# potamides/DeTikZify

Hardware: NVIDIA H100
Metric: TikZ tokens/sec/GPU (decode, 384px cond, 2k ctx) (higher is better)
Workload: dtype bf16

## Files before the change

### detikzify_b200/csrc/decode_mega.cu

```cuda
#include "common.cuh"
#include "fp8.cuh"
#include "launch.h"

namespace dtk {
namespace {

constexpr int NCW = 8;
constexpr int NPW = 4;
constexpr int MEGA_THREADS = (NCW + NPW) * 32;
constexpr int CONSUMER_THREADS = NCW * 32;
static_assert(NCW % NPW == 0, "slot ownership: NPW must divide NCW");
constexpr int TILE_BYTES = 8192;
constexpr int KV_V_OFF = 4096;
constexpr int NT = 104;
constexpr int NS = 72;
constexpr int NG = 48;
constexpr long long SPIN_CYCLES = 4000000000ll;

DTK_DEV void mbar_init(uint32_t bar, uint32_t count) {
  asm volatile("mbarrier.init.shared::cta.b64 [%0], %1;\n" ::"r"(bar), "r"(count));
}
DTK_DEV void mbar_expect_tx(uint32_t bar, uint32_t bytes) {
  asm volatile("mbarrier.arrive.expect_tx.shared::cta.b64 _, [%0], %1;\n" ::"r"(bar), "r"(bytes) : "memory");
}
DTK_DEV void mbar_arrive(uint32_t bar) {
  asm volatile("mbarrier.arrive.shared::cta.b64 _, [%0];\n" ::"r"(bar) : "memory");
}
DTK_DEV uint32_t mbar_try(uint32_t bar, uint32_t parity) {
  uint32_t done;
  asm volatile(
      "{\n\t.reg .pred p;\n\t"
      "mbarrier.try_wait.parity.shared::cta.b64 p, [%1], %2;\n\t"
      "selp.u32 %0, 1, 0, p;\n\t}\n"
      : "=r"(done)
      : "r"(bar), "r"(parity)
      : "memory");
  return done;
}
DTK_DEV void mbar_wait_slow(uint32_t bar, uint32_t parity) {
  uint32_t spins = 0;
  long long t0 = 0;
  while (!mbar_try(bar, parity)) {
    if ((++spins & 1023u) == 0) {
      const long long now = clock64();
      if (t0 == 0) t0 = now;
      else if (now - t0 > SPIN_CYCLES) __trap();
    }
  }
}
DTK_DEV void mbar_wait(uint32_t bar, uint32_t parity) {
  if (!mbar_try(bar, parity)) mbar_wait_slow(bar, parity);
}
DTK_DEV void bulk_g2s(uint32_t dst, const void* src, uint32_t bytes, uint32_t bar) {
  asm volatile("cp.async.bulk.shared::cluster.global.mbarrier::complete_tx::bytes [%0], [%1], %2, [%3];\n" ::"r"(dst),
               "l"(src), "r"(bytes), "r"(bar)
               : "memory");
}
DTK_DEV void bulk_g2s_hint(uint32_t dst, const void* src, uint32_t bytes, uint32_t bar, uint64_t pol) {
  asm volatile("cp.async.bulk.shared::cluster.global.mbarrier::complete_tx::bytes.L2::cache_hint [%0], [%1], %2, [%3], %4;\n" ::"r"(dst),
               "l"(src), "r"(bytes), "r"(bar), "l"(pol)
               : "memory");
}
DTK_DEV uint64_t policy_evict_first() {
  uint64_t pol;
  asm volatile("createpolicy.fractional.L2::evict_first.b64 %0, 1.0;\n" : "=l"(pol));
  return pol;
}
DTK_DEV void consumer_sync() { asm volatile("bar.sync 1, %0;\n" ::"n"(CONSUMER_THREADS) : "memory"); }

typedef unsigned long long u64;
DTK_DEV void st_tag(u64* p, float v, uint32_t tag) {
  const u64 w = ((u64)tag << 32) | (u64)__float_as_uint(v);
  asm volatile("st.relaxed.gpu.global.u64 [%0], %1;\n" ::"l"(p), "l"(w) : "memory");
}
DTK_DEV ulonglong2 ld_strong2(const u64* p) {
  ulonglong2 r;
  asm volatile("ld.relaxed.gpu.global.v2.u64 {%0, %1}, [%2];\n" : "=l"(r.x), "=l"(r.y) : "l"(p) : "memory");
  return r;
}
DTK_DEV ulonglong2 ld_weak2(const u64* p) {
  ulonglong2 r;
  asm volatile("ld.global.cg.v2.u64 {%0, %1}, [%2];\n" : "=l"(r.x), "=l"(r.y) : "l"(p) : "memory");
  return r;
}
DTK_DEV u64 ld_strong1(const u64* p) {
  u64 r;
  asm volatile("ld.relaxed.gpu.global.u64 %0, [%1];\n" : "=l"(r) : "l"(p) : "memory");
  return r;
}
DTK_DEV u64 ld_weak1(const u64* p) {
  u64 r;
  asm volatile("ld.global.cg.u64 %0, [%1];\n" : "=l"(r) : "l"(p) : "memory");
  return r;
}
DTK_DEV bool tag_ok(u64 w, uint32_t tag) { return (uint32_t)(w >> 32) == tag; }
DTK_DEV float tag_val(u64 w) { return __uint_as_float((uint32_t)w); }
struct Spin {
  uint32_t n = 0;
  long long t0 = 0;
  DTK_DEV void tick() {
    __nanosleep(32);
    if ((++n & 255u) == 0) {
      const long long now = clock64();
      if (t0 == 0) t0 = now;
      else if (now - t0 > SPIN_CYCLES) __trap();
    }
  }
};
DTK_DEV u64 poll1(const u64* p, uint32_t tag) {
  Spin sp;
  for (;;) {
    const u64 w = ld_strong1(p);
    if (tag_ok(w, tag)) return w;
    sp.tick();
  }
}
DTK_DEV float settle1(u64 w, const u64* p, uint32_t tag, bool nowait) {
  if (!tag_ok(w, tag) && !nowait) w = poll1(p, tag);
  return tag_val(w);
}

template <int N>
DTK_DEV void ld_pairs(const u64* const (&ptr)[N], const bool (&on)[N], uint32_t tag, bool nowait, float2 (&out)[N]) {
  ulonglong2 w[N];
#pragma unroll
  for (int u = 0; u < N; ++u)
    if (on[u]) w[u] = ld_weak2(ptr[u]);
  Spin sp;
  for (;;) {
    bool bad[N], any = false;
#pragma unroll
    for (int u = 0; u < N; ++u) {
      bad[u] = on[u] && !(tag_ok(w[u].x, tag) && tag_ok(w[u].y, tag));
      any = any || bad[u];
    }
    if (!any || nowait) break;
    sp.tick();
#pragma unroll
    for (int u = 0; u < N; ++u)
      if (bad[u]) w[u] = ld_strong2(ptr[u]);
  }
#pragma unroll
  for (int u = 0; u < N; ++u) out[u] = on[u] ? make_float2(tag_val(w[u].x), tag_val(w[u].y)) : make_float2(0.f, 0.f);
}

enum { PH_QKV = 0, PH_ATTN = 1, PH_O = 2, PH_GU = 3, PH_DOWN = 4, PH_LM = 5 };

struct AttnSplit {
  int active, head, j0, j1, last;
  int cph;
  int n_items;
// ... 50 lines not shown
        if (bad[u]) w[u] = ld_strong2(src + 2 * (ks * 128 + u * 32 + lane));
    }
#pragma unroll
    for (int u = 0; u < 4; ++u) v[u] = on[u] ? make_float2(tag_val(w[u].x), tag_val(w[u].y)) : make_float2(0.f, 0.f);
  } else {
#pragma unroll
    for (int u = 0; u < 4; ++u) {
      v[u] = make_float2(0.f, 0.f);
      if (on[u]) {
        const uint32_t e = *reinterpret_cast<const uint32_t*>(src_bf16 + 2 * (ks * 128 + u * 32 + lane));
        v[u] = make_float2(__uint_as_float(e << 16), __uint_as_float(e & 0xffff0000u));
      }
    }
  }
  float ss = 0.f;
#pragma unroll
  for (int u = 0; u < 4; ++u) {
    float a = v[u].x, b = v[u].y;
    if (norm_w) {
      ss += a * a + b * b;
      a *= __uint_as_float(gw[u] << 16);
      b *= __uint_as_float(gw[u] & 0xffff0000u);
    }
    const float ah = __bfloat162float(__float2bfloat16_rn(a)), bh = __bfloat162float(__float2bfloat16_rn(b));
    const uint32_t hi = pack_bf16x2(ah, bh), lo = pack_bf16x2(a - ah, b - bh);
    const uint32_t hi2 = __shfl_xor_sync(0xffffffffu, hi, 4), lo2 = __shfl_xor_sync(0xffffffffu, lo, 4);
    if (!(lane & 4)) xb[(size_t)(ks * 16 + u * 4 + (lane >> 3)) * 4 + (lane & 3)] = make_uint4(hi, hi2, lo, lo2);
  }
  if (norm_w) {
    ss = warp_sum(ss);
    if (lane == 0) slice_ss[ks] = ss;
  }
  __syncwarp();
  if (lane == 0) {
    __threadfence_block();
    slice_tag[ks] = my_tag;
  }
  __syncwarp();
}
DTK_DEV float slices_rn(const float* slice_ss, int nslice, int K, float eps) {
  const int lane = threadIdx.x & 31;
  float t = 0.f;
  for (int i = lane; i < nslice; i += 32) t += *reinterpret_cast<const volatile float*>(slice_ss + i);
  t = warp_sum(t);
  return rsqrtf(t / K + eps);
}

template <bool DBG, int HD, bool F8>
__global__ void __launch_bounds__(MEGA_THREADS, 1) decode_mega_kernel(const MegaArgs p) {
  constexpr int HALF = HD / 2;
  constexpr int LPK = HD / 8;
  constexpr int NGRP = 32 / LPK;
  constexpr int NST = NCW * NGRP;
  constexpr int PS = HD + 4;
  constexpr int PPL = HD / 64;
  constexpr int HSH = HD == 128 ? 7 : 6;
  extern __shared__ __align__(128) uint8_t smem[];
  const int tid = threadIdx.x, lane = tid & 31, warp = tid >> 5;
  const int c = blockIdx.x, G = gridDim.x;
  const int nslots = p.nslots;
  uint8_t* ring = smem;
  float* actf = reinterpret_cast<float*>(smem + (size_t)nslots * TILE_BYTES);
  uint4* xb = reinterpret_cast<uint4*>(actf);
  uint64_t* bars = reinterpret_cast<uint64_t*>(actf + p.act_floats);
  float* red = reinterpret_cast<float*>(bars + 2 * nslots);
  float* rope_s = red + 16;
  float* tpart = rope_s + 128;
  int* gcnt = reinterpret_cast<int*>(tpart + NT * 16);
  float* rbuf = reinterpret_cast<float*>(gcnt + NG);
  float* qkn = rbuf + NG * 16;
  float* slice_ss = qkn + 384;
  uint32_t* slice_tag = reinterpret_cast<uint32_t*>(slice_ss + NS);
  const uint32_t full0 = smem_u32(bars), empty0 = smem_u32(bars + nslots);
  const uint32_t ring_u32 = smem_u32(ring);

  if (tid == 0) {
    for (int s = 0; s < nslots; ++s) {
      mbar_init(full0 + 8 * s, 1);
      mbar_init(empty0 + 8 * s, 1);
    }
    asm volatile("fence.mbarrier_init.release.cluster;\n" ::: "memory");
    asm volatile("fence.proxy.async.shared::cta;\n" ::: "memory");
  }
  const int pos = p.pos[0], slot = p.slots[0];
  int tok = p.tok[0];
  if (tok < 0 || tok >= p.V) tok = 0;
  const int qd = p.heads * HD, kd = p.kv_heads * HD;
  if (tid < NS) slice_tag[tid] = (uint32_t)p.bar_base[1];
  if (tid < HD) rope_s[tid] = p.rope_cs[(int64_t)pos * HD + tid];
  __syncthreads();
  const AttnSplit as = attn_split(p, c, G, pos);
  const int kvh = as.head / (p.heads / p.kv_heads);
  const bf16* kv_slot = p.kv + (int64_t)slot * p.kv_slot_stride;
  const int shlen = p.share_len[0];
  const bf16* kv_share = p.kv + (int64_t)p.share_slot[0] * p.kv_slot_stride;
  const int nphase = 5 * p.L + 1;

  struct Walk {
    uint32_t nb = 0;
    uint32_t gb = 0;
    uint32_t rot = 0;
  };
  auto phase_span = [&](const Walk& w, const MegaMat& m, int& g0, int& cnt, int& nact) {
    nact = m.nact;
    int ci = c + G - (int)w.rot;
    if (ci >= G) ci -= G;
    g0 = ci * m.per;
    cnt = (ci < nact) ? min(m.per, m.groups - g0) : 0;
  };
  auto mat_of = [](int ph) { return ph == PH_QKV ? 0 : ph == PH_O ? 1 : ph == PH_GU ? 2 : ph == PH_DOWN ? 3 : 4; };

  if (warp >= NCW) {
    asm volatile("setmaxnreg.dec.sync.aligned.u32 56;\n");
    const uint32_t pw = (uint32_t)(warp - NCW);
    if (lane == 0) {
      const bool evf = !(p.variant & 1);
      const uint64_t pol = policy_evict_first();
      Walk w;
      uint32_t sl = pw, use = 0;
      long long* tr = nullptr;
      uint32_t tr_nb0 = 0;
      int l = 0, ph = 0;
      for (int it = 0; it < nphase; ++it) {
        if (it == nphase - 1) { ph = PH_LM; l = 0; }
        if (DBG && ph == 0) {
          tr = (p.dbg2 && l == p.dbg_layer && it != nphase - 1) ? p.dbg2 + (int64_t)c * MEGA_DBG2_ROWS * 4 : nullptr;
          if (tr) tr_nb0 = w.nb;
        }
        const bool attn = ph == PH_ATTN;
        const MegaMat& m = p.mat[mat_of(ph)];
        int g0 = 0, cnt = 0, nact = 0;
        if (!attn) phase_span(w, m, g0, cnt, nact);
        const int tpg = attn ? 1 : m.tpg;
        const int ntiles = attn ? as.n_items : cnt * tpg;
        const int64_t kvo = (int64_t)l * p.kv_layer_stride + (int64_t)kvh * p.max_len * HD;
        const bf16* base = attn ? kv_slot + kvo
                                : m.base + (int64_t)l * m.layer_stride + (int64_t)g0 * tpg * MEGA_TILE_ELEMS;
        uint32_t j = (pw + NPW - (w.nb & (NPW - 1))) & (NPW - 1);
        MegaF8 f8{};
        uint32_t jk = 0, jks = j;
        if (F8) {
          if (!attn && ph != PH_LM) f8 = p.f8[mat_of(ph)];
          while (jks >= (uint32_t)tpg) { jks -= tpg; ++jk; }
        }
        if ((int)j < ntiles) {
          for (; (int)j < ntiles; j += NPW) {
            if (use > 0) mbar_wait(empty0 + 8 * sl, (use - 1) & 1);
            const uint32_t dst = ring_u32 + sl * TILE_BYTES, fb = full0 + 8 * sl;
            if (attn) {
              const int key0 = as.j0 + (int)j * 16;
              const uint32_t bytes = (uint32_t)min(16, p.max_len - key0) * (uint32_t)(HD * 2);
              const bf16* kb = (key0 < shlen ? kv_share + kvo : base) + (int64_t)key0 * HD;
              mbar_expect_tx(fb, 2 * bytes);
              bulk_g2s(dst, kb, bytes, fb);
              bulk_g2s(dst + KV_V_OFF, kb + p.kv_v_offset, bytes, fb);
            } else if (F8 && ph != PH_LM) {
              mbar_expect_tx(fb, MEGA_F8_TILE_BYTES + 16);
              const uint8_t* src = f8.tiles + (int64_t)l * f8.layer_stride + ((int64_t)g0 * tpg + j) * MEGA_F8_TILE_BYTES;
              if (evf) bulk_g2s_hint(dst, src, MEGA_F8_TILE_BYTES, fb, pol);
              else bulk_g2s(dst, src, MEGA_F8_TILE_BYTES, fb);
              bulk_g2s(dst + MEGA_F8_TILE_BYTES, f8.exps + (int64_t)l * f8.exp_stride + (int64_t)(g0 + (int)jk) * 16, 16, fb);
            } else {
              mbar_expect_tx(fb, TILE_BYTES);
              if (evf) bulk_g2s_hint(dst, base + (int64_t)j * MEGA_TILE_ELEMS, TILE_BYTES, fb, pol);
              else bulk_g2s(dst, base + (int64_t)j * MEGA_TILE_ELEMS, TILE_BYTES, fb);
            }
            if (DBG && tr) {
              const uint32_t row = w.nb + j - tr_nb0;
              if (row < 160u) tr[row * 4] = clock64();
            }
            sl += NPW;
            if (sl >= (uint32_t)nslots) { sl -= nslots; ++use; }
            if (F8) {
              jks += NPW;
              while (jks >= (uint32_t)tpg) { jks -= tpg; ++jk; }
            }
          }
        }
        w.nb += ntiles;
        if (!attn) {
          w.gb += cnt;
          w.rot += (uint32_t)nact;
          if (w.rot >= (uint32_t)G) w.rot -= G;
        }
        if (++ph == 5) { ph = 0; ++l; }
      }
    }
    return;
  }

  asm volatile("setmaxnreg.inc.sync.aligned.u32 224;\n");
  const int dflags = DBG ? p.dbg_flags : 0;
  const bool nowait = (dflags & 2) != 0;
  unsigned long long bar_target = p.bar_base[0];
  const uint32_t epoch = (uint32_t)p.bar_base[1];
  Walk w;
  uint32_t sl = (uint32_t)warp, use = 0;
  uint32_t cur_slot = 0;
  auto release = [&]() {
    __syncwarp();
    if (lane == 0) mbar_arrive(empty0 + 8 * cur_slot);
  };
  long long* dbg = (DBG && p.dbg) ? p.dbg + (int64_t)c * nphase * 4 : nullptr;
  long long* ctr = nullptr;
  uint32_t ctr_nb0 = 0;
  int it = 0, l = 0, ph = 0;
  auto stamp = [&](int k) {
    if (!DBG) return;
    if (dbg && tid == 0) {
      unsigned long long t;
      asm volatile("mov.u64 %0, %%globaltimer;\n" : "=l"(t));
      dbg[it * 4 + k] = (long long)t;
    }
    if (ctr && tid == 0 && ph < 5) ctr[(160 + ph) * 4 + k] = clock64();
  };

  u64* const t_xa = p.tg;
  u64* const t_xb = t_xa + p.tg_H;
  u64* const t_q = t_xb + p.tg_H;
  u64* const t_kn = t_q + qd;
  u64* const t_vn = t_kn + kd;
  u64* const t_att = t_vn + kd;
  u64* const t_h = t_att + qd;
  u64* const t_part = t_h + p.tg_I;

  float best_v = -INFINITY;
  int best_i = 0x7fffffff;
  for (it = 0; it < nphase; ++it) {
    if (it == nphase - 1) { ph = PH_LM; l = 0; }
    const uint32_t tag = epoch + (uint32_t)it + 1u;
    if (DBG && ph == 0) {
      ctr = (p.dbg2 && l == p.dbg_layer && it != nphase - 1) ? p.dbg2 + (int64_t)c * MEGA_DBG2_ROWS * 4 : nullptr;
      ctr_nb0 = w.nb;
    }
    stamp(0);
    if (ph == PH_ATTN) {
      if (as.active) {
        const int hw = lane >> (HSH - 3), l16 = lane & (LPK - 1);
        if (warp == 0) {
          const float sl2 = (HD == 128 ? 0.08838834764831845f : 0.125f) * 1.4426950408889634f;
          float2* q2 = reinterpret_cast<float2*>(qkn);
          const bool lastr = as.last != 0;
          const u64* ptr[3 * PPL];
          bool on[3 * PPL];
#pragma unroll
          for (int u = 0; u < PPL; ++u) {
            ptr[u] = t_q + as.head * HD + 2 * (lane + 32 * u);
            ptr[PPL + u] = t_kn + kvh * HD + 2 * (lane + 32 * u);
            ptr[2 * PPL + u] = t_vn + kvh * HD + 2 * (lane + 32 * u);
            on[u] = true;
            on[PPL + u] = lastr;
            on[2 * PPL + u] = lastr;
          }
          float2 v[3 * PPL];
          ld_pairs<3 * PPL>(ptr, on, tag - 1, nowait, v);
#pragma unroll
          for (int u = 0; u < PPL; ++u) {
            q2[lane + 32 * u] = make_float2(v[u].x * sl2, v[u].y * sl2);
            if (lastr) { q2[HALF + lane + 32 * u] = v[PPL + u]; q2[HD + lane + 32 * u] = v[2 * PPL + u]; }
          }
        }
        consumer_sync();
        stamp(1);
        float q[8];
        {
          const float4 a = *reinterpret_cast<const float4*>(qkn + l16 * 8), b = *reinterpret_cast<const float4*>(qkn + l16 * 8 + 4);
          q[0] = a.x; q[1] = a.y; q[2] = a.z; q[3] = a.w; q[4] = b.x; q[5] = b.y; q[6] = b.z; q[7] = b.w;
        }
        float m = -INFINITY, lsum = 0.f, o[8];
#pragma unroll
        for (int i = 0; i < 8; ++i) o[i] = 0.f;
        auto keys4 = [&](const uint4 (&kr)[4], const uint4 (&vr)[4], const bool (&valid)[4]) {
          float s2[4];
#pragma unroll
          for (int u = 0; u < 4; ++u) {
            float kf[8];
            unpack8(kr[u], kf);
            float d = 0.f;
#pragma unroll
            for (int i = 0; i < 8; ++i) d += q[i] * kf[i];
            s2[u] = d;
          }
#pragma unroll
          for (int st = LPK / 2; st > 0; st >>= 1)
#pragma unroll
            for (int u = 0; u < 4; ++u) s2[u] += __shfl_xor_sync(0xffffffffu, s2[u], st);
          float mx = m;
#pragma unroll
          for (int u = 0; u < 4; ++u) { s2[u] = valid[u] ? s2[u] : -INFINITY; mx = fmaxf(mx, s2[u]); }
          if (mx == -INFINITY) return;
          const float alpha = exp2f(m - mx);
          float pj[4], ps = 0.f;
#pragma unroll
          for (int u = 0; u < 4; ++u) { pj[u] = exp2f(s2[u] - mx); ps += pj[u]; }
          lsum = lsum * alpha + ps;
#pragma unroll
          for (int i = 0; i < 8; ++i) o[i] *= alpha;
#pragma unroll
          for (int u = 0; u < 4; ++u) {
            if (valid[u]) {
              float vf[8];
              unpack8(vr[u], vf);
#pragma unroll
              for (int i = 0; i < 8; ++i) o[i] += pj[u] * vf[i];
            }
          }
          m = mx;
        };
        {
          uint32_t j = ((uint32_t)warp + NCW - (w.nb & (NCW - 1))) & (NCW - 1);
          if ((int)j < as.n_items) {
            for (; (int)j < as.n_items; j += NCW) {
// ... 398 lines not shown
  const int64_t tile = q >> 8;
  const int ks = (int)(tile % tpg), gi = (int)(tile / tpg);
  uint32_t out[4];
#pragma unroll
  for (int h = 0; h < 4; ++h) {
    uint32_t word = 0;
#pragma unroll
    for (int u = 0; u < 2; ++u) {
      const int m = 2 * (h & 1) + u;
      const int ar = (m & 1) * 8 + (lane >> 2);
      const int row = tile_row(mode, hd, gi, ar);
      const int col = ks * 256 + (2 * p + (h >> 1)) * 16 + (m >> 1) * 8 + 2 * (lane & 3);
      uint32_t codes = 0;
      if (row < N && col < K) {
        const float inv = pow2f(-exps[gi * 16 + ar]);
        const float2 v = __bfloat1622float2(*reinterpret_cast<const __nv_bfloat162*>(src + (int64_t)row * K + col));
        codes = float2_to_e4m3x2(v.x * inv, v.y * inv);
      }
      word |= codes << (16 * u);
    }
    out[h] = word;
  }
  *reinterpret_cast<uint4*>(dst + q * 16) = make_uint4(out[0], out[1], out[2], out[3]);
}

}

int64_t mega_tiled_elems(int N, int K, int mode, int* groups, int* tpg) {
  int g = (mode == TILE_GLU) ? (N / 2 + 7) / 8 : (N + 15) / 16;
  int t = (K + 255) / 256;
  if (groups) *groups = g;
  if (tpg) *tpg = t;
  return (int64_t)g * t * MEGA_TILE_ELEMS;
}

cudaError_t launch_retile(const bf16* src, int N, int K, int mode, int hd, bf16* dst, cudaStream_t s) {
  if ((K & 7) || (mode == TILE_ROPE && ((hd != 64 && hd != 128) || N % hd))) return cudaErrorInvalidValue;
  int groups, tpg;
  mega_tiled_elems(N, K, mode, &groups, &tpg);
  const int64_t chunks = (int64_t)groups * tpg * 512;
  retile_kernel<<<(unsigned)((chunks + 255) / 256), 256, 0, s>>>(src, N, K, mode, hd, groups, tpg, dst);
  return cudaGetLastError();
}

cudaError_t launch_retile_f8(const bf16* src, int N, int K, int mode, int hd, uint8_t* dst, int8_t* exps, unsigned int* bad,
                             cudaStream_t s) {
  if ((K & 7) || (mode == TILE_ROPE && ((hd != 64 && hd != 128) || N % hd))) return cudaErrorInvalidValue;
  int groups, tpg;
  mega_tiled_elems(N, K, mode, &groups, &tpg);
  f8_rows_kernel<<<(unsigned)((groups * 16 + 7) / 8), 256, 0, s>>>(src, N, K, mode, hd, groups, exps, bad);
  const int64_t chunks = (int64_t)groups * tpg * 256;
  f8_tile_kernel<<<(unsigned)((chunks + 255) / 256), 256, 0, s>>>(src, N, K, mode, hd, groups, tpg, exps, dst);
  return cudaGetLastError();
}

int mega_smem_bytes(const MegaArgs& a) {
  return a.nslots * TILE_BYTES + a.act_floats * 4 + 2 * a.nslots * 8 + (16 + 128 + NT * 16) * 4 + NG * 4 + NG * 16 * 4 + 384 * 4 + NS * 8;
}

cudaError_t mega_configure(MegaArgs& a, int H, int I, int heads, int hd, int max_smem_optin, int num_sms, int* grid_out) {
  if (hd != 64 && hd != 128) return cudaErrorInvalidValue;
  a.hd = hd;
  auto pad = [](int k) { return (k + 255) / 256 * 256; };
  int actf = pad(H) > pad(I) ? pad(H) : pad(I);
  if (pad(heads * hd) > actf) actf = pad(heads * hd);
  const int nst = NCW * (256 / hd), merge = 2 * nst + nst * hd + 16 * (hd + 4);
  if (actf < merge) actf = merge;
  actf = (actf + 31) & ~31;
  a.act_floats = actf;
  a.tg_H = pad(H);
  a.tg_I = pad(I);
  if ((I + 255) / 256 > NT - 44 || (I + 255) / 256 > NS || (H + 255) / 256 > NS) return cudaErrorInvalidValue;
  const int fixed = actf * 4 + (16 + 128 + NT * 16) * 4 + NG * 4 + NG * 16 * 4 + 384 * 4 + NS * 8 + 64;
  int nslots = (max_smem_optin - fixed) / (TILE_BYTES + 16);
  if (nslots > 32) nslots = 32;
  nslots &= ~(NCW - 1);
  if (nslots < NCW) return cudaErrorInvalidValue;
  a.nslots = nslots;
  if (heads > num_sms) return cudaErrorInvalidValue;
  *grid_out = num_sms;
  return cudaSuccess;
}

cudaError_t launch_decode_mega(const MegaArgs& a, int grid, cudaStream_t s, uint64_t* counter) {
  const int smem = mega_smem_bytes(a);
  const bool dbgk = a.dbg != nullptr || a.dbg2 != nullptr || a.dbg_flags != 0;
  const void* fn;
  const bool f8 = a.f8[0].tiles != nullptr;
  if (a.hd == 128 && !f8) fn = dbgk ? (const void*)decode_mega_kernel<true, 128, false> : (const void*)decode_mega_kernel<false, 128, false>;
  else if (a.hd == 64 && !f8) fn = dbgk ? (const void*)decode_mega_kernel<true, 64, false> : (const void*)decode_mega_kernel<false, 64, false>;
  else if (a.hd == 128) fn = dbgk ? (const void*)decode_mega_kernel<true, 128, true> : (const void*)decode_mega_kernel<false, 128, true>;
  else if (a.hd == 64) fn = dbgk ? (const void*)decode_mega_kernel<true, 64, true> : (const void*)decode_mega_kernel<false, 64, true>;
  else return cudaErrorInvalidValue;
  cudaError_t e = cudaFuncSetAttribute(fn, cudaFuncAttributeMaxDynamicSharedMemorySize, smem);
  if (e != cudaSuccess) return e;
  void* args[] = {(void*)&a};
  e = cudaLaunchCooperativeKernel(fn, dim3(grid), dim3(MEGA_THREADS), args, (size_t)smem, s);
  if (counter) ++*counter;
  return e;
}

}
```

### detikzify_b200/csrc/engine.cu

```cuda
#include <cuda_runtime.h>

#include <chrono>
#include <cmath>
#include <cstdio>
#include <cstdlib>
#include <cstring>
#include <map>
#include <string>
#include <thread>
#include <vector>

#include "../../include/detikzify_b200.h"
#include "launch.h"

using namespace dtk;

namespace {

struct WEntry {
  std::string name;
  int rows, cols;
  uint64_t offset, nbytes;
};

// ... 495 lines not shown
  g.bias = W(eng, "proj.b"); g.out_f32 = out; g.ldo = c.hidden;
  DTK_CK(launch_gemm(g, s, &eng->launches));
  return DTK_OK;
}

bf16* kv_layer(dtk_engine* eng, int slot, int layer) {
  return eng->kv + (int64_t)slot * eng->kv_slot_stride + (int64_t)layer * eng->kv_layer_stride;
}

int mega_layer_tiles(dtk_engine* eng, bool fp8) {
  static const char* names[4] = {"wqkv", "wo", "wgu", "wd"};
  const dtk_config& c = eng->cfg;
  MegaArgs& m = eng->mega;
  const int hd = c.head_dim, L = c.layers;
  const int64_t esz = fp8 ? 1 : 2;
  int64_t per_layer = 0, off[4], exp_layer = 0, eoff[4];
  for (int i = 0; i < 4; ++i) {
    off[i] = per_layer;
    per_layer += (int64_t)m.mat[i].groups * m.mat[i].tpg * MEGA_TILE_ELEMS * esz;
    eoff[i] = exp_layer;
    exp_layer += (int64_t)m.mat[i].groups * 16;
  }
  const int64_t tiles_bytes = per_layer * L, exp0 = tiles_bytes, bad0 = (exp0 + exp_layer * L + 255) / 256 * 256;
  const int64_t total = fp8 ? bad0 + 4 * (int64_t)L * 4 : tiles_bytes;
  DTK_CK(cudaDeviceSynchronize());
  uint8_t* buf = nullptr;
  DTK_ALLOC(buf, total);
  unsigned int* bad = reinterpret_cast<unsigned int*>(buf + bad0);
  cudaError_t e = fp8 ? cudaMemset(bad, 0, 4 * (size_t)L * sizeof(unsigned int)) : cudaSuccess;
  for (int l = 0; l < L && e == cudaSuccess; ++l)
    for (int i = 0; i < 4 && e == cudaSuccess; ++i) {
      const MegaMat& mm = m.mat[i];
      const bf16* src = W(eng, LN("dec.L", l, names[i]));
      uint8_t* dst = buf + (int64_t)l * per_layer + off[i];
      e = fp8 ? launch_retile_f8(src, mm.N, mm.K, mm.mode, hd, dst, reinterpret_cast<int8_t*>(buf + exp0 + (int64_t)l * exp_layer + eoff[i]),
                                 bad + l * 4 + i, 0)
              : launch_retile(src, mm.N, mm.K, mm.mode, hd, reinterpret_cast<bf16*>(dst), 0);
    }
  if (e == cudaSuccess) e = cudaDeviceSynchronize();
  std::vector<unsigned int> nbad(fp8 ? 4 * L : 0);
  if (e == cudaSuccess && fp8) e = cudaMemcpy(nbad.data(), bad, nbad.size() * sizeof(unsigned int), cudaMemcpyDeviceToHost);
  if (e != cudaSuccess) {
    cudaFree(buf);
    eng->err = std::string("decode tiles: ") + cudaGetErrorString(e);
    return DTK_ERR_CUDA;
  }
  for (size_t k = 0; k < nbad.size(); ++k)
    if (nbad[k]) {
      cudaFree(buf);
      eng->err = "invalid argument: decode_fp8: layer " + std::to_string(k / 4) + " " + names[k % 4] + " holds " +
                 std::to_string(nbad[k]) + " values that are not an e4m3 value times a power-of-two row scale (quantize the "
                 "weights first: load(..., quantize=\"fp8\"))";
      return DTK_ERR_INVALID;
    }
  for (auto& g : eng->graphs) cudaGraphExecDestroy(g.second);
  eng->graphs.clear();
  cudaFree(eng->d_tiled);
  cudaFree(eng->d_tiled8);
  eng->d_tiled = fp8 ? nullptr : reinterpret_cast<bf16*>(buf);
  eng->d_tiled8 = fp8 ? buf : nullptr;
  for (int i = 0; i < 4; ++i) {
    m.mat[i].base = fp8 ? nullptr : reinterpret_cast<const bf16*>(buf + off[i]);
    m.mat[i].layer_stride = fp8 ? 0 : per_layer / 2;
    m.f8[i] = fp8 ? MegaF8{buf + off[i], reinterpret_cast<const int8_t*>(buf + exp0 + eoff[i]), per_layer, exp_layer} : MegaF8{};
  }
  eng->decode_fp8 = fp8 ? 1 : 0;
  return DTK_OK;
}

uint64_t decode_weight_bytes(const dtk_config& c, bool fp8) {
  const uint64_t H = c.hidden, I = c.inter, V = c.vocab, qd = (uint64_t)c.heads * c.head_dim, kd = (uint64_t)c.kv_heads * c.head_dim;
  const uint64_t layer_w = (uint64_t)c.layers * ((qd + 2 * kd) * H + H * qd + 3 * H * I);
  const uint64_t layer_rows = (uint64_t)c.layers * ((qd + 2 * kd) + H + 2 * I + H);
  return (fp8 ? layer_w + layer_rows : 2 * layer_w) + 2 * V * H;
}

int nsplit_for(const dtk_config& c, int B) {
  int n = (2 * 132 + c.heads * B - 1) / (c.heads * B);
  if (n < 1) n = 1;
  if (n > 16) n = 16;
  return n;
}

int decode_launches(dtk_engine* eng, int B, const int64_t* tok64, float* logits, cudaStream_t s) {
  const dtk_config& c = eng->cfg;
  const int H = c.hidden, I = c.inter, HD = c.head_dim, qd = c.heads * HD, kd = c.kv_heads * HD;
  const float scale = 1.0f / sqrtf((float)HD);
  uint64_t* lc = &eng->launches;
  if (B == 1 && eng->decode_impl == 1 && eng->mega_ok) {
    if (tok64) {
      tok64_to_32_kernel<<<1, 32, 0, s>>>(tok64, eng->d_tok, 1);
      ++*lc;
      DTK_CK(cudaGetLastError());
    }
    MegaArgs m = eng->mega;
    m.logits = logits;
    m.dbg = eng->mega_debug ? eng->d_dbg : nullptr;
    m.dbg_flags = eng->mega_flags;
    m.variant = eng->mega_variant;
    if (eng->mega_nslots >= 8 && eng->mega_nslots < m.nslots) m.nslots = eng->mega_nslots & ~7;
    m.fuse_greedy = 0;
    if (eng->gen_fused && logits == eng->d_logits) {
      m.fuse_greedy = 1; m.bad_token = eng->gen_sample.bad_token; m.ring = eng->ring; m.max_pos = eng->cfg.max_len - 1;
      m.amax = eng->d_amax; m.gen_tok = eng->d_tok; m.gen_pos = eng->d_pos; m.gen_step = eng->d_gen; m.host_ring = eng->dev_ring;
    }
    m.dbg2 = (eng->mega_debug && eng->mega_trace_layer >= 0) ? eng->d_dbg2 : nullptr;
    m.dbg_layer = eng->mega_trace_layer;
    DTK_CK(launch_decode_mega(m, eng->mega_grid, s, lc));
    return DTK_OK;
  }
  DTK_CK(launch_embed_tokens(tok64 ? nullptr : eng->d_tok, tok64, B, W(eng, "dec.embed"), H, c.vocab, eng->d_x, s, lc));
  int nsplit = nsplit_for(c, B);
  if (eng->decode_gemm_min_batch > 0 && B >= eng->decode_gemm_min_batch && B <= c.max_len) {
    if (eng->cas_len > 0 && eng->cas_slot >= 0 && nsplit > 4) nsplit = 4;
    const int qkvd = qd + 2 * kd;
    const bool fp8 = eng->decode_fp8 != 0 && B < 64;
    auto gemm = [&](const bf16* A, int K, const bf16* Wm, int N, const float* resid, int glu, float* o32, bf16* o16, int ldo,
                    int l = 0, int mat = -1) {
      GemmArgs g{};
      g.A = A; g.lda = K; g.W = Wm; g.ldw = K; g.M = B; g.N = N; g.K = K;
      g.resid = resid; g.ldr = ldo; g.glu = glu; g.out_f32 = o32; g.out_bf16 = o16; g.ldo = ldo;
      if (fp8 && mat >= 0) {
        const MegaMat& mm = eng->mega.mat[mat];
        const MegaF8& t = eng->mega.f8[mat];
        const GemmF8 w{t.tiles + l * t.layer_stride, t.exps + l * t.exp_stride, mm.groups, mm.tpg, mm.mode, HD};
        return launch_gemm_swap_f8(g, w, s, lc);
      }
      return launch_gemm(g, s, lc);
    };
    const bool cas = eng->cas_len > 0 && eng->cas_slot >= 0;
    const int ctiles_all = cas ? (eng->cas_len + 63) / 64 : 0;
    const int cslots = 16 - nsplit;
    const int ctile = cas ? std::max(2, (ctiles_all + cslots - 1) / cslots) : 0;
    const int csplit = cas ? (ctiles_all + ctile - 1) / ctile : 0;
    for (int l = 0; l < c.layers; ++l) {
      DTK_CK(launch_rmsnorm(eng->d_x, H, W(eng, LN("dec.L", l, "norm1")), c.rms_eps, B, H, eng->p_xn, s, lc));
      DTK_CK(gemm(eng->p_xn, H, W(eng, LN("dec.L", l, "wqkv")), qkvd, nullptr, 0, eng->p_qkv, nullptr, qkvd, l, 0));
      DTK_CK(launch_rope_kv_decode(eng->p_qkv, B, eng->d_slots, eng->d_pos, c.heads, c.kv_heads, eng->rope_cs, eng->d_q,
                                   kv_layer(eng, 0, l), eng->kv_slot_stride, eng->kv_v_offset, c.max_len, HD, s, lc, cas ? eng->p_q : nullptr));
      if (cas) {
        AttnArgs f{};
        f.q = eng->p_q; f.k = kv_layer(eng, eng->cas_slot, l); f.v = f.k + eng->kv_v_offset;
        f.q_bs = 0; f.q_hs = HD; f.q_rs = qd;
        f.k_bs = 0; f.k_hs = (int64_t)c.max_len * HD; f.k_rs = HD;
        f.v_bs = 0; f.v_hs = (int64_t)c.max_len * HD; f.v_rs = HD;
        f.B = 1; f.heads = c.heads; f.kv_group = c.heads / c.kv_heads; f.Tq = B; f.Tk = eng->cas_len; f.q_pos0 = 0;
        f.causal = 0; f.head_dim = HD; f.scale = scale;
        f.part_o = eng->d_part_o; f.part_ml = eng->d_part_ml; f.part_np = nsplit + csplit; f.part_idx0 = nsplit; f.part_tiles = ctile;
        DTK_CK(launch_flash_attn(f, s, lc));
      }
      {
        DecodeAttnArgs a{};
        a.q = eng->d_q; a.q_stride = qd; a.kv_base = kv_layer(eng, 0, l); a.kv_slot_stride = eng->kv_slot_stride;
        a.kv_v_offset = eng->kv_v_offset; a.slots = eng->d_slots; a.pos = eng->d_pos; a.share_slot = eng->d_share_slot; a.share_len = eng->d_share_len;
        a.B = B; a.heads = c.heads; a.kv_group = c.heads / c.kv_heads; a.max_len = c.max_len; a.nsplit = nsplit;
        a.head_dim = HD; a.scale = scale;
        a.part_o = eng->d_part_o; a.part_ml = eng->d_part_ml; a.counters = eng->d_counters;
        a.out = eng->d_att; a.out_stride = qd; a.out_bf16 = eng->p_att;
        if (cas) { a.key_begin = eng->cas_len; a.np = nsplit + csplit; }
        DTK_CK(launch_decode_attn(a, s, lc));
      }
      DTK_CK(gemm(eng->p_att, qd, W(eng, LN("dec.L", l, "wo")), H, eng->d_x, 0, eng->d_x, nullptr, H, l, 1));
      DTK_CK(launch_rmsnorm(eng->d_x, H, W(eng, LN("dec.L", l, "norm2")), c.rms_eps, B, H, eng->p_xn, s, lc));
      DTK_CK(gemm(eng->p_xn, H, W(eng, LN("dec.L", l, "wgu")), 2 * I, nullptr, 1, nullptr, eng->p_h, I, l, 2));
      DTK_CK(gemm(eng->p_h, I, W(eng, LN("dec.L", l, "wd")), H, eng->d_x, 0, eng->d_x, nullptr, H, l, 3));
    }
    DTK_CK(launch_rmsnorm(eng->d_x, H, W(eng, "dec.norm"), c.rms_eps, B, H, eng->p_xn, s, lc));
    DTK_CK(gemm(eng->p_xn, H, W(eng, "dec.lm_head"), c.vocab, nullptr, 0, logits, nullptr, c.vocab));
    return DTK_OK;
  }
  for (int l = 0; l < c.layers; ++l) {
    {
      GemvArgs g{};
      g.mode = GEMV_QKV; g.W = W(eng, LN("dec.L", l, "wqkv")); g.N = qd + 2 * kd; g.K = H;
      g.x = eng->d_x; g.x_stride = H; g.norm_w = W(eng, LN("dec.L", l, "norm1")); g.eps = c.rms_eps;
      g.out = eng->d_q; g.out_stride = qd; g.B = B;
      g.slots = eng->d_slots; g.pos = eng->d_pos; g.rope_cs = eng->rope_cs;
      g.kv_base = kv_layer(eng, 0, l); g.kv_slot_stride = eng->kv_slot_stride; g.kv_v_offset = eng->kv_v_offset;
      g.q_dim = qd; g.kv_dim = kd; g.max_len = c.max_len; g.head_dim = HD;
      DTK_CK(launch_gemv(g, s, lc));
    }
    {
      DecodeAttnArgs a{};
      a.q = eng->d_q; a.q_stride = qd; a.kv_base = kv_layer(eng, 0, l); a.kv_slot_stride = eng->kv_slot_stride;
      a.kv_v_offset = eng->kv_v_offset; a.slots = eng->d_slots; a.pos = eng->d_pos; a.share_slot = eng->d_share_slot; a.share_len = eng->d_share_len;
      a.B = B; a.heads = c.heads; a.kv_group = c.heads / c.kv_heads; a.max_len = c.max_len; a.nsplit = nsplit;
      a.head_dim = HD; a.scale = scale;
      a.part_o = eng->d_part_o; a.part_ml = eng->d_part_ml; a.counters = eng->d_counters;
      a.out = eng->d_att; a.out_stride = qd;
      DTK_CK(launch_decode_attn(a, s, lc));
    }
// ... 713 lines not shown
int dtk_gen_begin(dtk_engine* eng, const int* slots, const int* positions, const int64_t* first_ids_host, int B,
                  const dtk_sampling* params, const uint32_t* seq_ids, void* stream) {
  if (!eng) return DTK_ERR_INVALID;
  const dtk_config& c = eng->cfg;
  DTK_REQUIRE(slots && positions && first_ids_host && params, "null pointer");
  DTK_REQUIRE(B > 0 && B <= c.max_batch, "B exceeds max_batch");
  DTK_CK(cudaSetDevice(eng->device));
  cudaStream_t s = (cudaStream_t)stream;
  StateArgs st{};
  st.n = B; st.have_tok = 1;
  for (int i = 0; i < B; ++i) {
    DTK_REQUIRE(slots[i] >= 0 && slots[i] < c.max_seqs, "slot");
    DTK_REQUIRE(positions[i] >= 0 && positions[i] < c.max_len, "position exceeds max_len");
    DTK_REQUIRE(positions[i] >= eng->share_len[slots[i]] && positions[i] >= eng->shared_upto[slots[i]], "position lies inside a shared prefix");
    st.slots[i] = slots[i]; st.pos[i] = positions[i]; st.tok[i] = first_ids_host[i];
    st.share_slot[i] = eng->share_base[slots[i]] >= 0 ? eng->share_base[slots[i]] : slots[i];
    st.share_len[i] = eng->share_len[slots[i]];
  }
  set_cascade(eng, st);
  set_state_kernel<<<1, 64, 0, s>>>(st, eng->d_slots, eng->d_pos, eng->d_tok, eng->d_share_slot, eng->d_share_len);
  reset_gen_kernel<<<1, 1, 0, s>>>(eng->d_gen, eng->d_counters + (int64_t)c.max_batch * c.heads, params->seed);
  eng->launches += 2;
  DTK_CK(cudaGetLastError());
  DTK_CK(cudaStreamSynchronize(s));
  std::memset(eng->host_ring, 0, (size_t)eng->ring * 64 * sizeof(unsigned long long));

  eng->gen_B = B;
  eng->gen_params = *params;
  eng->gen_stream = s;
  {
    SampleArgs& a = eng->gen_sample;
    fill_sample_args(eng, a, eng->d_logits, B, *params);
    for (int i = 0; i < B; ++i) { a.seq[i].suppress = 0; a.seq[i].step = 1; a.seq[i].seq_id = seq_ids ? seq_ids[i] : (uint32_t)i; }
    a.gen_tok = eng->d_tok; a.gen_pos = eng->d_pos; a.gen_step = eng->d_gen; a.seed_dev = eng->d_gen + 1; a.seed = 0;
    a.host_ring = eng->dev_ring; a.ring = eng->ring;
    a.done_counter = eng->d_counters + (int64_t)c.max_batch * c.heads;
  }
  eng->gen_mega = (B == 1 && eng->decode_impl == 1 && eng->mega_ok);
  eng->gen_fused = eng->gen_mega && eng->fuse_greedy && !eng->gen_sample.do_sample;
  if (eng->gen_mega) {
    eng->gen_graph = nullptr;
    return DTK_OK;
  }
  char key[256];
  std::snprintf(key, sizeof(key), "B%d|t%.9g|p%.17g|k%d|s%d|b%d|e%d", B, (double)params->temperature,
                (double)params->top_p, params->top_k, params->do_sample, params->bad_token, params->begin_suppress_token);
  std::string skey(key);
  skey += "|g" + std::to_string(eng->decode_gemm_min_batch) + "|i" + std::to_string(get_gemm_impl());
  skey += "|c" + std::to_string(eng->cas_slot) + ":" + std::to_string(eng->cas_len);
  if (seq_ids) for (int i = 0; i < B; ++i) skey += "," + std::to_string(seq_ids[i]);
  auto it = eng->graphs.find(skey);
  if (it == eng->graphs.end()) {
    cudaGraph_t graph = nullptr;
    uint64_t before = eng->launches;
    if (!eng->cap_stream) DTK_CK(cudaStreamCreateWithFlags(&eng->cap_stream, cudaStreamNonBlocking));
    cudaStream_t cs = eng->cap_stream;
    DTK_CK(cudaStreamBeginCapture(cs, cudaStreamCaptureModeThreadLocal));
    int r = decode_launches(eng, B, nullptr, eng->d_logits, cs);
    if (r == DTK_OK) {
      cudaError_t e = launch_sample(eng->gen_sample, cs, &eng->launches);
      if (e != cudaSuccess) { eng->err = std::string("launch_sample: ") + cudaGetErrorString(e); r = DTK_ERR_CUDA; }
    }
    cudaError_t ce = cudaStreamEndCapture(cs, &graph);
    eng->launches = before;
    if (r != DTK_OK) { if (graph) cudaGraphDestroy(graph); return r; }
    if (ce != cudaSuccess) { eng->err = std::string("cudaStreamEndCapture: ") + cudaGetErrorString(ce); return DTK_ERR_CUDA; }
    cudaGraphExec_t exec = nullptr;
    DTK_CK(cudaGraphInstantiate(&exec, graph, 0));
    cudaGraphDestroy(graph);
    if (eng->graphs.size() >= 64) {
      for (auto& g : eng->graphs) cudaGraphExecDestroy(g.second);
      eng->graphs.clear();
    }
    it = eng->graphs.emplace(skey, exec).first;
  }
  eng->gen_graph = it->second;
  return DTK_OK;
}

int dtk_gen_step(dtk_engine* eng, void* stream) {
  if (!eng) return DTK_ERR_INVALID;
  DTK_REQUIRE(eng->gen_B > 0, "dtk_gen_begin not called");
  if (eng->gen_mega) {
    int r = decode_launches(eng, 1, nullptr, eng->d_logits, (cudaStream_t)stream);
    if (r != DTK_OK) return r;
    if (!eng->gen_fused) DTK_CK(launch_sample(eng->gen_sample, (cudaStream_t)stream, &eng->launches));
    return DTK_OK;
  }
  DTK_REQUIRE(eng->gen_graph != nullptr, "dtk_gen_begin not called");
  DTK_CK(cudaGraphLaunch(eng->gen_graph, (cudaStream_t)stream));
  const bool gemm_path = eng->decode_gemm_min_batch > 0 && eng->gen_B >= eng->decode_gemm_min_batch;
  eng->launches += gemm_path ? (uint64_t)eng->cfg.layers * (9 + (eng->cas_len > 0 ? 1 : 0)) + 4 : (uint64_t)eng->cfg.layers * 5 + 3;
  return DTK_OK;
}

int dtk_gen_wait(dtk_engine* eng, int64_t step, int32_t* tokens_out_host) {
  if (!eng) return DTK_ERR_INVALID;
  DTK_REQUIRE(eng->gen_B > 0 && step >= 0 && tokens_out_host, "gen state/step/out");
  volatile const unsigned long long* row = eng->host_ring + (size_t)(step % eng->ring) * eng->gen_B;
  const unsigned long long want = (unsigned long long)(step + 1);
  auto t0 = std::chrono::steady_clock::now();
  uint64_t spins = 0;
  for (int i = 0; i < eng->gen_B; ++i) {
    unsigned long long e;
    while (((e = row[i]) >> 32) != want) {
      if ((e >> 32) > want) {
        eng->err = "token ring overrun: dtk_gen_wait lagged more than the ring depth behind dtk_gen_step";
        return DTK_ERR_INVALID;
      }
      if ((++spins & 0x3ff) == 0) {
        cudaError_t q = cudaStreamQuery(eng->gen_stream);
        if (q != cudaSuccess && q != cudaErrorNotReady) {
          eng->err = std::string("stream error while waiting for token: ") + cudaGetErrorString(q);
          return DTK_ERR_CUDA;
        }
        if (q == cudaSuccess && (row[i] >> 32) != want) {
          eng->err = "stream idle but requested step was never launched";
          return DTK_ERR_INVALID;
        }
        if (std::chrono::steady_clock::now() - t0 > std::chrono::seconds(60)) {
          eng->err = "timeout waiting for generated token";
          return DTK_ERR_CUDA;
        }
      }
    }
    tokens_out_host[i] = (int32_t)(uint32_t)(e & 0xffffffffull);
  }
  return DTK_OK;
}

int dtk_gen_end(dtk_engine* eng) {
  if (!eng) return DTK_ERR_INVALID;
  if (eng->gen_B > 0) {
    DTK_CK(cudaSetDevice(eng->device));
    DTK_CK(cudaStreamSynchronize(eng->gen_stream));
  }
  eng->gen_graph = nullptr;
  eng->gen_mega = false;
  eng->gen_fused = false;
  eng->gen_B = 0;
  return DTK_OK;
}

int dtk_set_option(dtk_engine* eng, const char* key, int64_t value) {
  if (!eng || !key) return DTK_ERR_INVALID;
  DTK_REQUIRE(eng->gen_B == 0, "options cannot change inside a generation loop");
  if (std::strcmp(key, "decode_impl") == 0) {
    DTK_REQUIRE(value == 0 || value == 1, "decode_impl must be 0 (per-op) or 1 (persistent)");
    eng->decode_impl = (int)value;
    return DTK_OK;
  }
  if (std::strcmp(key, "decode_gemm_min_batch") == 0) {
    DTK_REQUIRE(value >= 0 && value <= 64, "decode_gemm_min_batch must be in 0..64");
    eng->decode_gemm_min_batch = (int)value;
    return DTK_OK;
  }
  if (std::strcmp(key, "gemm_impl") == 0) {
    DTK_REQUIRE(value >= 0 && value <= 2, "gemm_impl must be 0..2");
    set_gemm_impl((int)value);
    return DTK_OK;
  }
  if (std::strcmp(key, "cascade_attn") == 0) {
    eng->cascade_attn = value ? 1 : 0;
    return DTK_OK;
  }
  if (std::strcmp(key, "gemm_swap_split") == 0) {
    DTK_REQUIRE(value >= 0 && value <= 8, "gemm_swap_split must be 0 (heuristic) .. 8");
// ... 187 lines not shown
```

### detikzify_b200/csrc/launch.h

```cpp
#pragma once
#include <cuda_bf16.h>
#include <cuda_runtime.h>
#include <stdint.h>

typedef __nv_bfloat16 bf16;

namespace dtk {

enum { ACT_NONE = 0, ACT_GELU_TANH = 1, ACT_GELU_ERF = 2 };

struct GemmArgs {
  const bf16* A;
  int64_t lda;
  int a_rows_per_batch;
  int64_t a_batch_stride;
  const bf16* W;
  int64_t ldw;
  int M, N, K;
  const bf16* bias;
  const bf16* rowbias;
  int rowbias_mod;
  const float* resid;
  int64_t ldr;
  int act;
// ... 122 lines not shown
  bf16* out_bf16;
};
cudaError_t launch_decode_attn(const DecodeAttnArgs& a, cudaStream_t s, uint64_t* counter);

struct SampleSeq {
  int suppress;
  uint32_t step;
  uint32_t seq_id;
};
struct SampleArgs {
  const float* logits;
  int B, V;
  float temperature, top_p;
  float top_p_limit;
  int top_k, do_sample, bad_token, bs_token;
  uint64_t seed;
  const unsigned long long* seed_dev;
  float* scratch;
  int want_probs;
  int64_t* out_ids;
  int* gen_tok;
  int* gen_pos;
  unsigned long long* gen_step;
  unsigned long long* host_ring;
  int ring;
  int max_pos;
  unsigned int* done_counter;
  SampleSeq seq[64];
};
cudaError_t launch_sample(const SampleArgs& a, cudaStream_t s, uint64_t* counter);
void set_sample_impl(int impl);
int get_sample_impl();

enum { TILE_SEQ = 0, TILE_ROPE = 1, TILE_GLU = 2 };
constexpr int MEGA_TILE_ELEMS = 4096;
constexpr int MEGA_DBG2_ROWS = 168;
struct MegaMat {
  const bf16* base;
  int64_t layer_stride;
  int N, K;
  int groups, tpg;
  int per, nact;
  int mode;
};
constexpr int MEGA_F8_TILE_BYTES = 4096;
struct MegaF8 {
  const uint8_t* tiles;
  const int8_t* exps;
  int64_t layer_stride;
  int64_t exp_stride;
};
struct MegaArgs {
  int H, I, L, heads, kv_heads, V, max_len;
  int hd;
  float eps;
  const bf16 *embed, *final_norm;
  const bf16 *norm1_0, *norm2_0;
  int64_t norm_stride;
  MegaMat mat[5];
  const int *tok, *pos, *slots;
  const int *share_slot, *share_len;
  bf16* kv;
  int64_t kv_slot_stride, kv_layer_stride, kv_v_offset;
  const float* rope_cs;
  float* logits;
  unsigned long long* tg;
  int tg_H, tg_I;
  unsigned int* head_cnt;
  unsigned long long *bar_count, *bar_base;
  int nslots, act_floats;
  int fuse_greedy, bad_token, ring, max_pos;
  unsigned long long* amax;
  int *gen_tok, *gen_pos;
  unsigned long long *gen_step, *host_ring;
  int variant;
  int dbg_flags;
  long long* dbg;
  long long* dbg2;
  int dbg_layer;
  MegaF8 f8[4];
};
int mega_smem_bytes(const MegaArgs& a);
cudaError_t mega_configure(MegaArgs& a, int H, int I, int heads, int hd, int max_smem_optin, int num_sms, int* grid_out);
cudaError_t launch_decode_mega(const MegaArgs& a, int grid, cudaStream_t s, uint64_t* counter);
int64_t mega_tiled_elems(int N, int K, int mode, int* groups, int* tpg);
cudaError_t launch_retile(const bf16* src, int N, int K, int mode, int hd, bf16* dst, cudaStream_t s);
cudaError_t launch_retile_f8(const bf16* src, int N, int K, int mode, int hd, uint8_t* dst, int8_t* exps, unsigned int* bad,
                             cudaStream_t s);

cudaError_t launch_image_preprocess(const uint8_t* rgb, int h, int w, int S, const int* bounds_h, const int* coef_h, int ksize_h,
                                    const int* bounds_v, const int* coef_v, int ksize_v, float rescale, const float* mean,
                                    const float* std, uint8_t* tmp, float* out, uint8_t* out_u8, cudaStream_t s, uint64_t* counter);

cudaError_t launch_pool_attn(const float* q, const bf16* kv, int B, int N, int D, int heads, float scale,
                             bf16* out, cudaStream_t s, uint64_t* counter);

}
```

Measured before the change: 929.8.

## Chain decode megakernel launches with programmatic dependent launch

Launches the persistent decode megakernel with programmatic stream serialization so the next step's kernel can start before the previous one finishes. Producer warps delay griddepcontrol.wait until the first attention phase, so weight tile prefetch for layer-0 QKV overlaps the previous step's tail. Consumer warps wait before reading pos/tok, and the kernel signals launch_dependents at the LM-head phase. This hides per-step launch latency and the ramp-up of weight streaming, at the cost of co-residency pressure with a cooperative grid and subtle ordering risks around shared state such as barriers and logits.

```diff
diff --git a/detikzify_b200/csrc/decode_mega.cu b/detikzify_b200/csrc/decode_mega.cu
--- a/detikzify_b200/csrc/decode_mega.cu
+++ b/detikzify_b200/csrc/decode_mega.cu
@@ -67,6 +67,8 @@
   return pol;
 }
 DTK_DEV void consumer_sync() { asm volatile("bar.sync 1, %0;\n" ::"n"(CONSUMER_THREADS) : "memory"); }
+DTK_DEV void grid_dep_wait() { asm volatile("griddepcontrol.wait;\n" ::: "memory"); }
+DTK_DEV void grid_dep_launch() { asm volatile("griddepcontrol.launch_dependents;\n" ::: "memory"); }
 
 typedef unsigned long long u64;
 DTK_DEV void st_tag(u64* p, float v, uint32_t tag) {
@@ -283,18 +285,9 @@
     asm volatile("fence.mbarrier_init.release.cluster;\n" ::: "memory");
     asm volatile("fence.proxy.async.shared::cta;\n" ::: "memory");
   }
-  const int pos = p.pos[0], slot = p.slots[0];
-  int tok = p.tok[0];
-  if (tok < 0 || tok >= p.V) tok = 0;
+  __syncthreads();
   const int qd = p.heads * HD, kd = p.kv_heads * HD;
-  if (tid < NS) slice_tag[tid] = (uint32_t)p.bar_base[1];
-  if (tid < HD) rope_s[tid] = p.rope_cs[(int64_t)pos * HD + tid];
-  __syncthreads();
-  const AttnSplit as = attn_split(p, c, G, pos);
-  const int kvh = as.head / (p.heads / p.kv_heads);
-  const bf16* kv_slot = p.kv + (int64_t)slot * p.kv_slot_stride;
-  const int shlen = p.share_len[0];
-  const bf16* kv_share = p.kv + (int64_t)p.share_slot[0] * p.kv_slot_stride;
+  const int kvh = (c % p.heads) / (p.heads / p.kv_heads);
   const int nphase = 5 * p.L + 1;
 
   struct Walk {
@@ -321,6 +314,7 @@
       uint32_t sl = pw, use = 0;
       long long* tr = nullptr;
       uint32_t tr_nb0 = 0;
+      int pos = 0;
       int l = 0, ph = 0;
       for (int it = 0; it < nphase; ++it) {
         if (it == nphase - 1) { ph = PH_LM; l = 0; }
@@ -328,7 +322,15 @@
           tr = (p.dbg2 && l == p.dbg_layer && it != nphase - 1) ? p.dbg2 + (int64_t)c * MEGA_DBG2_ROWS * 4 : nullptr;
           if (tr) tr_nb0 = w.nb;
         }
+        if (ph == PH_ATTN && l == 0) {
+          grid_dep_wait();
+          pos = p.pos[0];
+        }
         const bool attn = ph == PH_ATTN;
+        const AttnSplit as = attn ? attn_split(p, c, G, pos) : AttnSplit{};
+        const bf16* kv_slot = p.kv + (int64_t)(attn ? p.slots[0] : 0) * p.kv_slot_stride;
+        const int shlen = attn ? p.share_len[0] : 0;
+        const bf16* kv_share = p.kv + (int64_t)(attn ? p.share_slot[0] : 0) * p.kv_slot_stride;
         const MegaMat& m = p.mat[mat_of(ph)];
         int g0 = 0, cnt = 0, nact = 0;
         if (!attn) phase_span(w, m, g0, cnt, nact);
@@ -387,10 +389,19 @@
         if (++ph == 5) { ph = 0; ++l; }
       }
     }
+    grid_dep_launch();
     return;
   }
 
   asm volatile("setmaxnreg.inc.sync.aligned.u32 224;\n");
+  grid_dep_wait();
+  const int pos = p.pos[0], slot = p.slots[0];
+  int tok = p.tok[0];
+  if (tok < 0 || tok >= p.V) tok = 0;
+  const AttnSplit as = attn_split(p, c, G, pos);
+  if (tid < NS) slice_tag[tid] = (uint32_t)p.bar_base[1];
+  if (tid < HD) rope_s[tid] = p.rope_cs[(int64_t)pos * HD + tid];
+  consumer_sync();
   const int dflags = DBG ? p.dbg_flags : 0;
   const bool nowait = (dflags & 2) != 0;
   unsigned long long bar_target = p.bar_base[0];
@@ -428,7 +439,10 @@
   float best_v = -INFINITY;
   int best_i = 0x7fffffff;
   for (it = 0; it < nphase; ++it) {
-    if (it == nphase - 1) { ph = PH_LM; l = 0; }
+    if (it == nphase - 1) {
+      ph = PH_LM; l = 0;
+      grid_dep_launch();
+    }
     const uint32_t tag = epoch + (uint32_t)it + 1u;
     if (DBG && ph == 0) {
       ctr = (p.dbg2 && l == p.dbg_layer && it != nphase - 1) ? p.dbg2 + (int64_t)c * MEGA_DBG2_ROWS * 4 : nullptr;
@@ -993,7 +1007,7 @@
   return cudaSuccess;
 }
 
-cudaError_t launch_decode_mega(const MegaArgs& a, int grid, cudaStream_t s, uint64_t* counter) {
+cudaError_t launch_decode_mega(const MegaArgs& a, int grid, cudaStream_t s, uint64_t* counter, bool chain) {
   const int smem = mega_smem_bytes(a);
   const bool dbgk = a.dbg != nullptr || a.dbg2 != nullptr || a.dbg_flags != 0;
   const void* fn;
@@ -1006,7 +1020,19 @@
   cudaError_t e = cudaFuncSetAttribute(fn, cudaFuncAttributeMaxDynamicSharedMemorySize, smem);
   if (e != cudaSuccess) return e;
   void* args[] = {(void*)&a};
-  e = cudaLaunchCooperativeKernel(fn, dim3(grid), dim3(MEGA_THREADS), args, (size_t)smem, s);
+  cudaLaunchAttribute at[2];
+  at[0].id = cudaLaunchAttributeCooperative;
+  at[0].val.cooperative = 1;
+  at[1].id = cudaLaunchAttributeProgrammaticStreamSerialization;
+  at[1].val.programmaticStreamSerializationAllowed = 1;
+  cudaLaunchConfig_t cfg = {};
+  cfg.gridDim = dim3(grid);
+  cfg.blockDim = dim3(MEGA_THREADS);
+  cfg.dynamicSmemBytes = (size_t)smem;
+  cfg.stream = s;
+  cfg.attrs = at;
+  cfg.numAttrs = chain ? 2 : 1;
+  e = cudaLaunchKernelExC(&cfg, fn, args);
   if (counter) ++*counter;
   return e;
 }
diff --git a/detikzify_b200/csrc/engine.cu b/detikzify_b200/csrc/engine.cu
--- a/detikzify_b200/csrc/engine.cu
+++ b/detikzify_b200/csrc/engine.cu
@@ -601,7 +601,7 @@
   return n;
 }
 
-int decode_launches(dtk_engine* eng, int B, const int64_t* tok64, float* logits, cudaStream_t s) {
+int decode_launches(dtk_engine* eng, int B, const int64_t* tok64, float* logits, cudaStream_t s, bool chain = false) {
   const dtk_config& c = eng->cfg;
   const int H = c.hidden, I = c.inter, HD = c.head_dim, qd = c.heads * HD, kd = c.kv_heads * HD;
   const float scale = 1.0f / sqrtf((float)HD);
@@ -625,7 +625,7 @@
     }
     m.dbg2 = (eng->mega_debug && eng->mega_trace_layer >= 0) ? eng->d_dbg2 : nullptr;
     m.dbg_layer = eng->mega_trace_layer;
-    DTK_CK(launch_decode_mega(m, eng->mega_grid, s, lc));
+    DTK_CK(launch_decode_mega(m, eng->mega_grid, s, lc, chain && !tok64 && !(eng->mega_variant & 2)));
     return DTK_OK;
   }
   DTK_CK(launch_embed_tokens(tok64 ? nullptr : eng->d_tok, tok64, B, W(eng, "dec.embed"), H, c.vocab, eng->d_x, s, lc));
@@ -1505,7 +1505,7 @@
   if (!eng) return DTK_ERR_INVALID;
   DTK_REQUIRE(eng->gen_B > 0, "dtk_gen_begin not called");
   if (eng->gen_mega) {
-    int r = decode_launches(eng, 1, nullptr, eng->d_logits, (cudaStream_t)stream);
+    int r = decode_launches(eng, 1, nullptr, eng->d_logits, (cudaStream_t)stream, true);
     if (r != DTK_OK) return r;
     if (!eng->gen_fused) DTK_CK(launch_sample(eng->gen_sample, (cudaStream_t)stream, &eng->launches));
     return DTK_OK;
diff --git a/detikzify_b200/csrc/launch.h b/detikzify_b200/csrc/launch.h
--- a/detikzify_b200/csrc/launch.h
+++ b/detikzify_b200/csrc/launch.h
@@ -228,7 +228,7 @@
 };
 int mega_smem_bytes(const MegaArgs& a);
 cudaError_t mega_configure(MegaArgs& a, int H, int I, int heads, int hd, int max_smem_optin, int num_sms, int* grid_out);
-cudaError_t launch_decode_mega(const MegaArgs& a, int grid, cudaStream_t s, uint64_t* counter);
+cudaError_t launch_decode_mega(const MegaArgs& a, int grid, cudaStream_t s, uint64_t* counter, bool chain = false);
 int64_t mega_tiled_elems(int N, int K, int mode, int* groups, int* tpg);
 cudaError_t launch_retile(const bf16* src, int N, int K, int mode, int hd, bf16* dst, cudaStream_t s);
 cudaError_t launch_retile_f8(const bf16* src, int N, int K, int mode, int hd, uint8_t* dst, int8_t* exps, unsigned int* bad,
```

Result: no change. 931.8, median of 6 (+0.2%).
